# tardis-sn/stardis

Measured on AMD Instinct MI355X. Metric: spectral points/sec (N_nu x N_depth), higher is better.
Workload: dtype f64; 1 GPU; S-c2: solar MARCS structure, 6500-6600 A at R=500000, 2000 lines, fp64; scaling=one GPU, n_nu_global=7634, n_nu_per_gpu=7634, n_depth=56, n_lines=2000, n_theta=20, voigt_evaluations_global=16803184, parallelism=nu-shard x1, hip_graph=False, graph_steps_per_launch=1, syntheses_in_flight_per_gpu=1, line_inputs=dense, outputs=F_nu and total_alphas (N_d, N_nu); the optional alpha_line plane is not written

## Files before the change

stardis_amd/csrc/sdx_kernels.h:

```cpp
#pragma once
#include <type_traits>

#include "sdx_math.h"
#include "sdx_broadening.h"
#include "sdx_cheb.h"

namespace sdx {

constexpr int kBlock = 256;

__device__ __forceinline__ void wave_sync()
{
    __builtin_amdgcn_fence(__ATOMIC_RELEASE, "wavefront");
    __builtin_amdgcn_wave_barrier();
    __builtin_amdgcn_fence(__ATOMIC_ACQUIRE, "wavefront");
}


constexpr int kDnuPartials = 256;
constexpr int kGridSample = 2048;
constexpr int kGridSampleOffset = 512;
__device__ __forceinline__ void grid_sample_block(const int bid, const int n_blocks, int64_t n_nu, const double* __restrict__ nus, double* __restrict__ sample)
{
    const int64_t cstride = (n_nu + kGridSample - 1) / kGridSample;
// ... 159 lines not shown

__device__ __forceinline__ int64_t window_rule(int64_t c, int64_t n_nu, double d_nu, double r_dnu, double gamma, double dw, double alpha,
                                               int& lo, int& hi)
{
    const double pixels = mul_rn(div_by(mul_rn(add_rn(gamma, dw), alpha), d_nu, r_dnu), 20.0);
    const double forced = pixels > 10.0 ? pixels : 10.0;
    const int64_t hw = forced >= (double)n_nu ? n_nu : (int64_t)forced;
    const int64_t l = c - hw, h = c + hw;
    lo = (int)(l < 0 ? 0 : l);
    hi = (int)(h > n_nu ? n_nu : h);
    return hw;
}

constexpr int kPreDepths = 64;
constexpr int kPreBlock = 1024;

constexpr int kNarrowHalfWidth = 64;
constexpr int kNarrowReach = 128;
constexpr int kMediumHalfWidth = 4096;
constexpr int kMaxTile = 512;

#ifdef SDX_WALK_STATS
constexpr int kWalkStatSlots = 1 << 19;
__device__ unsigned long long g_walk_stats[(size_t)kWalkStatSlots * 8];
#endif
#ifdef SDX_PRE_STATS
constexpr int kPreStatSlots = 1 << 14;
__device__ unsigned long long g_pre_stats[(size_t)kPreStatSlots * 8];
#define SDX_PRE_STAMP(n) do { if (tid == 0) pst[n] = wall_clock64(); } while (0)
#else
#define SDX_PRE_STAMP(n) do { } while (0)
#endif
struct alignas(16) WideScan {
    int lo, hi, clo, chi;
};
struct alignas(16) WideRec {
    double lnu, inv, yk, cv, cd, spare;
};
struct alignas(16) WideSlow {
    double y, amp;
};
struct alignas(32) WideRec32 {
    float nuh, yk, inv, ncl, cv, cd, pad0, pad1;
};
struct LineWork {
    WideScan* wscan;
    WideRec* wrec;
    WideSlow* wslow;
    WideRec32* wrec32;
    unsigned char* nhw;
    int skip_unlisted_scan;
    double* n_inv;
    double* n_y;
    double* n_amp;
    int narrow_raw;
    float* n_inv32;
    float* n_y32;
    float* n_amp32;
    float2v* lnu32;
    int* cnt_ge;
    int* centre;
    int* nhw_max;
    int* whw_max;
    int* hlist;
    int* hcount;
    int* xlist;
    int* wlist;
    int* wrank;
    WideScan* hscan;
    const int* sel;
    int n_pix;
    int gather;
    int64_t shard_begin, shard_end;
    unsigned long long* evals;
    int* ticket;
    int front;
    int n_csplit;
    const int* far_range;
};

__device__ __forceinline__ int* wide_list_of(const LineWork& w, int64_t n_lines) { return w.whw_max + n_lines; }
__device__ __forceinline__ int* wide_list_counts(const LineWork& w) { return w.hcount + 16; }

__device__ __forceinline__ unsigned small_div_magic(int d) { return d > 1 ? 0xFFFFFFFFu / (unsigned)d + 1u : 0u; }
__device__ __forceinline__ int small_div(int k, unsigned magic) { return magic ? (int)__umulhi((unsigned)k, magic) : k; }

constexpr int kListMaxChunks = kGridSample - 8;
__device__ __forceinline__ void compact_wide_lines(const LineWork& w, const int64_t n_lines, unsigned long long* __restrict__ s_mask, const int tid)
{
    const int n_split = w.n_csplit;
    const int n_chunks = (int)((n_lines + 63) >> 6);
    const int wave = tid >> 6, lane = tid & 63;
    int* const s_tot = reinterpret_cast<int*>(s_mask + kListMaxChunks);
    int* const clist = wide_list_of(w, n_lines);
    int* const ccount = wide_list_counts(w);
    for (int q = wave; q < n_chunks; q += kPreBlock / 64) {
        const int64_t l = (int64_t)q * 64 + lane;
        const unsigned long long m = __ballot(l < n_lines && w.whw_max[l] > 0);
        if (lane == 0) s_mask[q] = m;
    }
    __syncthreads();
    auto below = [&](int s, int q) {
        int c = 0;
        for (int j = lane; s + j * n_split < q; j += 64) c += __popcll(s_mask[s + j * n_split]);
        for (int off = 32; off > 0; off >>= 1) c += __shfl_xor(c, off);
        return c;
    };
    if (wave < n_split) {
        const int t = below(wave, n_chunks);
        if (lane == 0) s_tot[wave] = t;
    }
    __syncthreads();
    for (int q = wave; q < n_chunks; q += kPreBlock / 64) {
        const int s = q % n_split;
        int base = below(s, q);
        for (int k = 0; k < s; ++k) base += s_tot[k];
        const unsigned long long m = s_mask[q];
        if ((m >> lane) & 1)
            clist[base + (int)__builtin_amdgcn_mbcnt_hi((unsigned)(m >> 32), __builtin_amdgcn_mbcnt_lo((unsigned)m, 0u))] = q * 64 + lane;
    }
    if (tid < n_split) {
        int off = 0;
        for (int k = 0; k < tid; ++k) off += s_tot[k];
        ccount[tid] = s_tot[tid];
        ccount[8 + tid] = off;
    }
}

template <bool GEN, int kPreLines, bool LIST = true>
__device__ __forceinline__ void prepass_block(const int bx, const int by, const int gy, int n_depth, int64_t n_nu, const double* __restrict__ nus,
                                                         const double* __restrict__ dnu_partial, int n_partial,
                                                         int64_t n_lines, const double* __restrict__ line_nus,
                                                         const double* __restrict__ doppler,
                                                         const double* __restrict__ gammas, int gamma_cols,
                                                         const double* __restrict__ alphas, LineWork w,
                                                         int* __restrict__ out_lo_ref, int* __restrict__ out_hi_ref,
                                                         int n_line_blocks, const LineParams& lp, const int tid = threadIdx.x)
{
    int gbx = -1;
    if (bx >= n_line_blocks) {
        if (bx >= n_line_blocks + w.n_pix) {
            if (!w.gather) return;
            gbx = bx - n_line_blocks - w.n_pix;
        } else {
            if (by == 0 && w.cnt_ge) {
                const int64_t pidx = (int64_t)(bx - n_line_blocks) * blockDim.x + tid;
                const bool needed = !w.sel || (pidx >= w.shard_begin - kMediumHalfWidth - 2 * kNarrowReach - kMaxTile &&
                                               pidx <= w.shard_end + kMediumHalfWidth + 2 * kNarrowReach + kMaxTile);
                if (pidx <= n_nu + 1 && needed) {
                    int64_t cnt;
                    if (pidx == 0) cnt = n_lines;
                    else if (pidx == n_nu + 1) cnt = 0;
                    else {
                        const double v = nus[pidx - 1];
                        int64_t lo = 0, hi = n_lines;
                        while (lo < hi) {
                            const int64_t mid = lo + ((hi - lo) >> 1);
                            if (line_nus[mid] <= v) lo = mid + 1; else hi = mid;
                        }
                        cnt = lo;
                    }
                    w.cnt_ge[pidx] = (int)cnt;
                }
            }
            return;
        }
    }
// ... 2900 lines not shown
        const double2* pP = sP + gi + gc - j0;
        const double* pR = sRT + th * rstride + gc - j0;
        const double2 q0 = pP[j0], q1 = pP[j0 + 1];
        double a1 = q1.y, s1 = q1.x;
        double d10 = q0.x - s1;
        double t0 = mul_rn(q0.y * a1, pR[j0]);
#pragma unroll
        for (int j = 0; j < LMAX; ++j) {
            c[j] = 1.0, e[j] = 0.0;
            if (j >= j0) {
                if (j < LMAX - 1 || seg < NS - 1) {
                    const double2 q2 = pP[j + 2];
                    const double s2 = q2.x, a2 = q2.y;
                    const double t1 = mul_rn(a1 * a2, pR[j + 1]);
                    const double d21 = s2 - s1;
                    redo |= rt_coef_fast<false>(t0, t1, d10, d21, s1, c[j], e[j], kc);
                    t0 = t1, d10 = -d21, s1 = s2, a1 = a2;
                } else {
                    redo |= rt_coef_fast<true>(t0, 0.0, d10, 0.0, s1, c[j], e[j], kc);
                }
                A *= c[j];
                B = fma(c[j], B, e[j]);
            }
        }
    }
    if (redo) {
        A = 1.0, B = 0.0;
        for (int j = j0; j < LMAX; ++j) {
            const int gap = gc + j - j0;
            const double s0 = sP[gi + gap].x, s1 = sP[gi + gap + 1].x;
            const double t0 = mul_rn(sP[gi + gap].y * sP[gi + gap + 1].y, sRT[th * rstride + gap]);
            double cj, ej;
            if (gap < n_gap - 1) {
                const double t1 = mul_rn(sP[gi + gap + 1].y * sP[gi + gap + 2].y, sRT[th * rstride + gap + 1]);
                rt_coef_reference<false>(t0, t1, s0 - s1, sP[gi + gap + 2].x - s1, s1, cj, ej);
            } else {
                rt_coef_reference<true>(t0, 0.0, s0 - s1, 0.0, s1, cj, ej);
            }
            A *= cj;
            B = fma(cj, B, ej);
#pragma unroll
            for (int k = 0; k < LMAX; ++k)
                if (k == j) c[k] = cj, e[k] = ej;
        }
    }
    sAB[(seg * 64 + lane) * 2] = A;
    sAB[(seg * 64 + lane) * 2 + 1] = B;
    __syncthreads();
    double inten = 0.0;
    for (int k = 0; k < seg; ++k) inten = fma(sAB[(k * 64 + lane) * 2], inten, sAB[(k * 64 + lane) * 2 + 1]);
    if (seg == 0) {
        if (valid && I_nus) I_nus[(size_t)i * theta_stride + th] = 0.0;
        if (valid && g == 0 && F) F[i] = 0.0;
    }
    double* fx = sFx + (size_t)seg * LMAX * gpw * G + (active ? grp * G + g : 0);
    double* ip = valid && I_nus ? I_nus + ((size_t)(g_lo + 1) * n_nu + i) * theta_stride + th : nullptr;
    const size_t istep = (size_t)n_nu * theta_stride;
#pragma unroll
    for (int j = 0; j < LMAX; ++j) {
        if (j >= j0) {
            inten = fma(c[j], inten, e[j]);
            if (ip) *ip = inten, ip += istep;
            if (active) fx[(j - j0) * gpw * G] = inten * wt;
        }
    }
    fx = sFx + (size_t)seg * LMAX * gpw * G;
    wave_sync();
    if (F) {
        const int half = (n_theta + 1) >> 1;
        for (int p = lane; p < 2 * count * gpw; p += 64) {
            const int h = p & 1, q = p >> 1;
            const int b = (int)(((float)q + 0.5f) * (1.0f / (float)gpw)), gq = q - b * gpw;
            const double* cc = fx + q * G + (h ? half : 0);
            const int cnt = h ? n_theta - half : half;
            double sum = 0.0;
            for (int t = 0; t < cnt; ++t) sum = add_rn(sum, cc[t]);
            const double other = __shfl_xor(sum, 1);
            const int64_t iq = i0 + gq;
            if (h == 0 && iq < n_nu) F[(size_t)(g_lo + b + 1) * fld + iq] = add_rn(sum, other);
        }
    }
}

template <int P>
__global__ __launch_bounds__(kRtBlock) void k_raytrace_cont(int n_depth, int64_t n_nu, int n_theta, int theta_stride, int G,
                                                          const double* __restrict__ nus, const double* __restrict__ temps,
                                                          const double* __restrict__ ray_dist, const double* __restrict__ wts,
                                                          double* __restrict__ F, int64_t fld, double* __restrict__ Fc, int64_t fcld,
                                                          double* __restrict__ I_nus, int inward, int gpw, FusedTotal ft)
{
    constexpr int kBatch = P == 1 ? 4 : 2;
    extern __shared__ double smem[];
    const int lane = threadIdx.x & 63, wave = __builtin_amdgcn_readfirstlane(threadIdx.x >> 6);
    const int grp = lane / G, g = lane - grp * G;
    const int TH = P * G;
    const int64_t i0 = ((int64_t)blockIdx.x * (kRtBlock / 64) + wave) * gpw;
    const int64_t i = i0 + grp;
    const bool active = grp < gpw;
    const bool valid = active && i < n_nu;
    const int64_t ic = i < n_nu ? i : n_nu - 1;
    const int n_gap = n_depth - 1;
    const int col = n_depth;
    double* wbase = smem + (size_t)wave * ((3 * gpw * col + 2 * kBatch * gpw * TH + 1) & ~1);
    double2* sP = (double2*)wbase;
    double* sC = wbase + 2 * gpw * col;
    double* sX = sC + gpw * col;
    double* sXc = sX + kBatch * gpw * TH;
    const double nu = nus[ic];

    if (active) {
        for (int d = g; d < n_depth; d += G) {
            const double ac = ft.cont[(size_t)d * ft.cld + ic];
            double a = ac;
            if (ft.planes) {
                double line = ft.planes[(size_t)d * ft.pld + ic];
                for (int sp = 1; sp < ft.n_planes; ++sp) line = add_rn(line, ft.planes[((size_t)sp * n_depth + d) * ft.pld + ic]);
                a = add_rn(a, line);
                if (valid && ft.line_out) ft.line_out[(size_t)d * ft.out_ld + i] = line;
            }
            for (int x = 0; x < ft.n_extra; ++x) a = add_rn(a, ft.extra[x][(size_t)d * ft.eld + ic]);
            if (valid && ft.total_out) ft.total_out[(size_t)d * ft.out_ld + i] = a;
            sP[grp * col + d] = double2{ft.source ? ft.source[(size_t)d * ft.sld + ic] : planck_staged(nu, temps[d]), sqrt(a)};
            sC[grp * col + d] = sqrt(ac);
        }
    }
    wave_sync();
    const RtConst kc = rt_const_literals();

    const int gi = (active ? grp : 0) * col;
    double inten[P], intc[P], wt[P];
    int th[P];
    bool on[P];
#pragma unroll
    for (int k = 0; k < P; ++k) {
        th[k] = min(g + k * G, n_theta - 1);
        on[k] = g + k * G < n_theta;
        inten[k] = 0.0, intc[k] = 0.0;
        wt[k] = on[k] ? wts[th[k]] : 0.0;
    }
    if (inward) {
        for (int gap = n_gap - 1; gap >= 0; --gap) {
            const int gm = gap > 0 ? gap - 1 : n_gap - 1;
            const int dm = gap > 0 ? gap - 1 : n_depth - 1;
            const double2 q0 = sP[gi + gap + 1], q1 = sP[gi + gap], q2 = sP[gi + dm];
            const double s0 = q0.x, s1 = q1.x, s2 = q2.x;
            const double mg = q1.y * q0.y, mm = sP[gi + gm].y * sP[gi + gm + 1].y;
            const double mgc = sC[gi + gap] * sC[gi + gap + 1], mmc = sC[gi + gm] * sC[gi + gm + 1];
#pragma unroll
            for (int k = 0; k < P; ++k) {
                const double rg = ray_dist[(size_t)gap * theta_stride + th[k]], rm = ray_dist[(size_t)gm * theta_stride + th[k]];
                const double tg = mul_rn(mg, rg), tm = mul_rn(mm, rm);
                const double tgc = mul_rn(mgc, rg), tmc = mul_rn(mmc, rm);
                double c, e, cc, ec;
                rt_coef<false>(tg, tm, s0 - s1, s2 - s1, s1, c, e, kc);
                rt_coef<false>(tgc, tmc, s0 - s1, s2 - s1, s1, cc, ec, kc);
                inten[k] = tm == 0.0 ? inten[k] : fma(c, inten[k], e);
                intc[k] = tmc == 0.0 ? intc[k] : fma(cc, intc[k], ec);
            }
        }
#pragma unroll
        for (int k = 0; k < P; ++k) {
            if (valid && I_nus && on[k]) I_nus[(size_t)i * theta_stride + th[k]] = inten[k];
            if (active) sX[grp * TH + k * G + g] = inten[k] * wt[k], sXc[grp * TH + k * G + g] = intc[k] * wt[k];
        }
        wave_sync();
        if (lane < gpw && i0 + lane < n_nu) {
// ... 235 lines not shown
```

stardis_amd/csrc/stardis_hip.hip:

```cpp
#include <hip/hip_runtime.h>

#include <algorithm>
#include <cmath>
#include <cstdio>
#include <cstdlib>
#include <cstring>
#include <map>
#include <mutex>
#include <string>
#include <unordered_map>
#include <vector>

#include <dlfcn.h>
#include <rccl/rccl.h>

#include <memory>
#include <thread>

#include "../../include/stardis_hip.h"
#include "sdx_kernels.h"

using namespace sdx;

namespace {
// ... 321 lines not shown
        fail(SDX_ERR_HIP, "hipSetDevice failed: no usable HIP device " + std::to_string(device));
        (void)hipGetLastError();
        return nullptr;
    }
    sdx_ctx* ctx = new sdx_ctx();
    ctx->device = device;
    if (hipDeviceGetAttribute(&ctx->n_cu, hipDeviceAttributeMultiprocessorCount, device) != hipSuccess || ctx->n_cu <= 0) ctx->n_cu = 256;
    if (stream) {
        ctx->stream = (hipStream_t)stream;
    } else {
        if (hipStreamCreateWithFlags(&ctx->stream, hipStreamNonBlocking) != hipSuccess) {
            fail(SDX_ERR_HIP, "hipStreamCreate failed");
            delete ctx;
            return nullptr;
        }
        ctx->own_stream = true;
    }
    hipEventCreate(&ctx->t0);
    hipEventCreate(&ctx->t1);
    return ctx;
}

void sdx_destroy(sdx_ctx* ctx)
{
    if (!ctx) return;
    hipSetDevice(ctx->device);
    hipStreamSynchronize(ctx->stream);
    for (auto& r : ctx->records) {
        hipEventDestroy(r.start);
        hipEventDestroy(r.stop);
    }
    for (auto e : ctx->event_pool) hipEventDestroy(e);
    if (ctx->cont_ws) hipFree(ctx->cont_ws);
    if (ctx->t0) hipEventDestroy(ctx->t0);
    if (ctx->t1) hipEventDestroy(ctx->t1);
    if (ctx->line_ws) hipFree(ctx->line_ws);
    if (ctx->small_ws) hipFree(ctx->small_ws);
    if (ctx->part_ws) hipFree(ctx->part_ws);
    if (ctx->far_ws) hipFree(ctx->far_ws);
    if (ctx->cnt_ws) hipFree(ctx->cnt_ws);
    if (ctx->io_dev) hipFree(ctx->io_dev);
    if (ctx->io_pin) hipHostFree(ctx->io_pin);
    if (ctx->xfer_pin) hipHostFree(ctx->xfer_pin);
    for (auto& b : ctx->free_blocks) hipFree(b.second);
    if (ctx->own_stream) hipStreamDestroy(ctx->stream);
    delete ctx;
}

int sdx_set_stream(sdx_ctx* ctx, void* stream)
{
    REQUIRE(ctx, "null context");
    HIP_TRY(hipStreamSynchronize(ctx->stream));
    if (ctx->own_stream) {
        hipStreamDestroy(ctx->stream);
        ctx->own_stream = false;
    }
    if (stream) {
        ctx->stream = (hipStream_t)stream;
    } else {
        HIP_TRY(hipStreamCreateWithFlags(&ctx->stream, hipStreamNonBlocking));
        ctx->own_stream = true;
    }
    return SDX_OK;
}

void* sdx_get_stream(sdx_ctx* ctx) { return ctx ? (void*)ctx->stream : nullptr; }

int sdx_set_int_option(sdx_ctx* ctx, const char* name, int64_t value)
{
    REQUIRE(ctx && name, "sdx_set_int_option: null pointer");
    if (std::strcmp(name, "indexed_min_lines") == 0) {
        ctx->indexed_min_lines = value;
        return SDX_OK;
    }
    if (std::strcmp(name, "prepass_ticket_min_blocks") == 0) {
        ctx->prepass_ticket_min_blocks = value;
        return SDX_OK;
    }
    if (std::strcmp(name, "mixed_precision") == 0) {
        ctx->mixed_precision = value ? 1 : 0;
        return SDX_OK;
    }
    if (std::strcmp(name, "segmented_raytrace") == 0) {
        ctx->segmented_raytrace = value < 0 ? -1 : (value ? 1 : 0);
        return SDX_OK;
    }
    if (std::strcmp(name, "far_field") == 0) {
        ctx->far_field = value < 0 ? -1 : (value ? 1 : 0);
        return SDX_OK;
    }
    if (std::strcmp(name, "wide_list") == 0) {
        ctx->wide_list = value < 0 ? -1 : (value ? 1 : 0);
        return SDX_OK;
    }
    if (std::strcmp(name, "narrow_records") == 0) {
        ctx->narrow_records = value < 0 ? -1 : (value ? 1 : 0);
        return SDX_OK;
    }
    return fail(SDX_ERR_ARG, std::string("unknown option ") + name);
}

static bool far_field_on(const sdx_ctx* ctx, int64_t n_nu_global);
int sdx_far_field_active(const sdx_ctx* ctx, int64_t n_nu_global)
{
    REQUIRE(ctx, "null context");
    return far_field_on(ctx, n_nu_global) ? 1 : 0;
}

int sdx_far_field_rule(int64_t* min_points, int* tile_points, int* near_points)
{
    if (min_points) *min_points = 32768;
    if (tile_points) *tile_points = kFarTile;
    if (near_points) *near_points = (int)(kFarRatio * (kFarTile / 2)) + kFarTile / 2;
    return SDX_OK;
}

int sdx_synchronize(sdx_ctx* ctx)
{
    REQUIRE(ctx, "null context");
    HIP_TRY(hipStreamSynchronize(ctx->stream));
    return SDX_OK;
}

constexpr size_t kBlockPoolLimit = (size_t)4 << 30;
static size_t block_capacity(size_t bytes)
{
    if (bytes <= 256) return 256;
    if (bytes >= ((size_t)1 << 20)) return (bytes + ((size_t)1 << 20) - 1) & ~(((size_t)1 << 20) - 1);
    size_t c = 256;
    while (c < bytes) c <<= 1;
    return c;
}

void* sdx_malloc(sdx_ctx* ctx, size_t bytes)
{
    if (!ctx) return nullptr;
    hipSetDevice(ctx->device);
    const size_t cap = block_capacity(bytes);
    std::lock_guard<std::mutex> lock(ctx->pool_mutex);
    auto it = ctx->free_blocks.lower_bound(cap);
    if (it != ctx->free_blocks.end() && it->first <= 2 * cap) {
        void* p = it->second;
        ctx->free_block_bytes -= it->first;
        ctx->live_blocks[p] = it->first;
        ctx->free_blocks.erase(it);
        return p;
    }
    void* p = nullptr;
    hipError_t e = hipMalloc(&p, cap);
    if (e != hipSuccess && !ctx->free_blocks.empty()) {
        hipStreamSynchronize(ctx->stream);
        for (auto& b : ctx->free_blocks) hipFree(b.second);
        ctx->free_blocks.clear();
        ctx->free_block_bytes = 0;
        e = hipMalloc(&p, cap);
    }
    if (e != hipSuccess) {
        fail(SDX_ERR_OOM, std::string("hipMalloc: ") + hipGetErrorString(e));
        return nullptr;
    }
    ctx->live_blocks[p] = cap;
    return p;
}

int sdx_free(sdx_ctx* ctx, void* ptr)
{
    REQUIRE(ctx, "null context");
// ... 185 lines not shown
    return SDX_OK;
}

int sdx_timer_stop(sdx_ctx* ctx, double* elapsed_ms)
{
    REQUIRE(ctx && elapsed_ms, "sdx_timer_stop: null pointer");
    HIP_TRY(hipEventRecord(ctx->t1, ctx->stream));
    HIP_TRY(hipEventSynchronize(ctx->t1));
    float ms = 0.f;
    HIP_TRY(hipEventElapsedTime(&ms, ctx->t0, ctx->t1));
    *elapsed_ms = ms;
    return SDX_OK;
}

int sdx_profile_enable(sdx_ctx* ctx, int on)
{
    REQUIRE(ctx, "null context");
    ctx->profile = on != 0;
    return SDX_OK;
}

int sdx_profile_reset(sdx_ctx* ctx)
{
    REQUIRE(ctx, "null context");
    HIP_TRY(hipStreamSynchronize(ctx->stream));
    for (auto& r : ctx->records) {
        ctx->event_pool.push_back(r.start);
        ctx->event_pool.push_back(r.stop);
    }
    ctx->records.clear();
    return SDX_OK;
}

int sdx_profile_get(sdx_ctx* ctx, const char* kernel, int64_t* launches, double* total_ms)
{
    REQUIRE(ctx && kernel && launches && total_ms, "sdx_profile_get: null pointer");
    HIP_TRY(hipStreamSynchronize(ctx->stream));
    int64_t n = 0;
    double tot = 0.0;
    for (auto& r : ctx->records) {
        if (std::strcmp(r.name, kernel) != 0) continue;
        float ms = 0.f;
        HIP_TRY(hipEventElapsedTime(&ms, r.start, r.stop));
        tot += ms;
        ++n;
    }
    *launches = n;
    *total_ms = tot;
    return SDX_OK;
}

int sdx_profile_variant(sdx_ctx* ctx, const char* kernel, char* out, int out_len)
{
    REQUIRE(ctx && kernel && out && out_len > 0, "sdx_profile_variant: null pointer");
    out[0] = 0;
    for (auto& r : ctx->records)
        if (std::strcmp(r.name, kernel) == 0 && r.variant) std::snprintf(out, (size_t)out_len, "%s", r.variant);
    return SDX_OK;
}

struct ContinuumJob {
    const sdx_continuum* cont;
    int64_t nu_begin, nu_count;
    double* plane;
};
struct ClassifyPhase {
    int phase;
    int64_t begin, count;
    double* m_max;
};

static const int kSegWaves = knob("SDX_RT_NS") && std::atoi(knob("SDX_RT_NS")) == 4 ? 4 : 8;
static const int kSegMax = kSegWaves == 4 ? 14 : 7;
static int lane_recip(int G)
{
    return 65536 / G + 1;
}
static size_t seg_lds_doubles(int n_depth, int nth)
{
    const int gpw = 64 / nth;
    return (size_t)kSegWaves * 128 + std::max((((size_t)nth * ((n_depth - 1) | 1) + 1) & ~(size_t)1) + (size_t)2 * gpw * n_depth, (size_t)kSegWaves * kSegMax * gpw * nth);
}
constexpr int64_t kSegLegacyWaves = (int64_t)3 * 4 * 256;
static bool use_segmented_raytrace(const sdx_ctx* ctx, int n_depth, int64_t n_nu_global, int n_theta, bool plain)
{
    static const int env_mode = knob("SDX_RT_SEG") ? std::atoi(knob("SDX_RT_SEG")) : -1;
    const int mode = ctx->segmented_raytrace >= 0 ? (int)ctx->segmented_raytrace : env_mode;
    if (mode == 0 || !plain || n_theta > 64) return false;
    if ((n_depth - 1 + kSegWaves - 1) / kSegWaves > kSegMax || seg_lds_doubles(n_depth, n_theta) * sizeof(double) > 64 * 1024) return false;
    if (mode == 1) return true;
    const int64_t legacy_waves = (n_nu_global + 64 / n_theta - 1) / (64 / n_theta);
    return legacy_waves < kSegLegacyWaves;
}

static void launch_line_lists(sdx_ctx* ctx, int64_t n_lines, LineWork& w, int pre_lines, const ClassSource* from_classification = nullptr)
{
    ClassSource cs{};
    if (from_classification) cs = *from_classification;
    else cs.whw_max = w.whw_max;
    w.hlist = w.whw_max + n_lines;
    w.wlist = w.hlist + n_lines;
    w.wrank = w.wlist + n_lines;
    w.xlist = w.sel ? w.wrank + n_lines + 1 : nullptr;
    const unsigned hb = (unsigned)((n_lines + kHlistBlock - 1) / kHlistBlock);
    int* block_cnt = w.hcount + 16;
    hipLaunchKernelGGL(k_hlist_count, dim3(hb), dim3(kHlistBlock), 0, ctx->stream, n_lines, cs, block_cnt, w.sel, pre_lines, w.ticket);
    hipLaunchKernelGGL(k_hlist_scatter, dim3(hb), dim3(kHlistBlock), 0, ctx->stream, n_lines, cs, (const int*)block_cnt, w.hlist,
                       w.wlist, w.wrank, w.hcount, w.xlist, w.sel, pre_lines);
}

static int line_prepass(sdx_ctx* ctx, int n_depth, int64_t n_nu, const double* nus, int64_t n_lines, const double* line_nus,
                        const double* doppler, const double* gammas, int gamma_cols, const double* alphas, bool fill_work,
                        int32_t* lo_ref, int32_t* hi_ref, LineWork* w_out, bool count_evals = true,
                        const ContinuumJob* job = nullptr, const LineParams* gen = nullptr, int64_t nu_begin = 0, int64_t nu_count = -1,
                        const ClassifyPhase* ph = nullptr, int wide_splits = 0)
{
    if (nu_count < 0) nu_count = n_nu;
    const LineParams lp = gen ? *gen : LineParams{};
    int n_partial = 0;
    const bool consumes_classified = ph && ph->phase == 2;
    if (!consumes_classified) ctx->classified.valid = false;
    int rc = ensure_small(ctx, kSmallHeader);
    if (rc) return rc;
    const bool scan_in_block = n_nu <= 16384;
    LineWork w{};
    int pre_lines = ((n_lines + 15) / 16) * ((n_depth + kPreDepths - 1) / kPreDepths) <= 2 * (int64_t)ctx->n_cu ? 16 : 32;
    static const bool no_cull_early = knob("SDX_NO_CULL") != nullptr;
    static const int pre_lines_env = knob("SDX_PRE_LINES") ? std::atoi(knob("SDX_PRE_LINES")) : 0;
    const bool will_cull = fill_work && !no_cull_early && n_lines >= ctx->indexed_min_lines && !count_evals && !gen && n_nu > 16384 && nu_count < n_nu;
    if (will_cull && !lo_ref && (n_lines + 31) / 32 < ctx->prepass_ticket_min_blocks)
        pre_lines = (pre_lines_env == 32 || pre_lines_env == 48) ? pre_lines_env : (n_depth <= 56 ? 54 : 48);
    const int n_line_blocks = (int)((n_lines + pre_lines - 1) / pre_lines);
    int n_pixel_blocks = 0;
    if (fill_work) {
        rc = ensure(ctx, &ctx->line_ws, &ctx->line_ws_bytes, line_ws_need(n_depth, n_lines));
        if (rc) return rc;
        ctx->cnt_ge_len = (size_t)(n_nu + 2 + 63) / 64 * 64;
        rc = ensure(ctx, &ctx->cnt_ws, &ctx->cnt_ws_bytes, (ctx->cnt_ge_len + 10 * (size_t)n_lines + 128 + 3 * ((size_t)n_lines / 1024 + 8) + 8) * sizeof(int));
        if (rc) return rc;
        w = carve(ctx, n_depth, n_lines);
        if (n_depth > kPreDepths) HIP_TRY(hipMemsetAsync(w.nhw_max, 0, (size_t)2 * n_lines * sizeof(int), ctx->stream));
        if (count_evals) HIP_TRY(hipMemsetAsync(w.evals, 0, sizeof(unsigned long long), ctx->stream));
        else w.evals = nullptr;
        n_pixel_blocks = (int)((n_nu + 2 + kPreBlock - 1) / kPreBlock);
    }
    w.sel = nullptr;
    w.gather = 0;
    w.ticket = nullptr;
    w.front = 0;
    const int64_t chunks_per_subset = wide_splits > 0 ? ((n_lines + 63) / 64 + wide_splits - 1) / wide_splits : 0;
    if (fill_work && wide_splits > 0 && (ctx->wide_list == 1 || (ctx->wide_list < 0 && chunks_per_subset >= kListAutoChunks)) &&
        !ctx->mixed_precision && n_lines > 0 && n_lines < ctx->indexed_min_lines && (n_lines + 63) / 64 <= kListMaxChunks) {
        w.n_csplit = wide_splits;
    }
    static const int narrow_records_env = knob("SDX_NARROW_RECORDS") ? std::atoi(knob("SDX_NARROW_RECORDS")) : -1;
    const int narrow_records = ctx->narrow_records >= 0 ? (int)ctx->narrow_records : narrow_records_env;
    const bool very_dense = 2 * n_lines >= 8 * n_nu;
    if (fill_work && !gen && !ctx->mixed_precision && n_lines >= ctx->indexed_min_lines && (narrow_records == 0 || (very_dense && narrow_records != 1))) {
        w.narrow_raw = gamma_cols > 1 ? n_depth : 1;
        w.n_inv = const_cast<double*>(doppler);
        w.n_y = const_cast<double*>(gammas);
        w.n_amp = const_cast<double*>(alphas);
    }
    w.skip_unlisted_scan = (fill_work && n_lines >= ctx->indexed_min_lines && n_depth <= kPreDepths) ? 1 : 0;
    w.n_pix = n_pixel_blocks;
    w.shard_begin = nu_begin;
    w.shard_end = nu_begin + nu_count;
    static const bool no_cull = knob("SDX_NO_CULL") != nullptr;
    const bool cull = fill_work && !no_cull && n_lines >= ctx->indexed_min_lines && !count_evals && !gen && !scan_in_block && nu_count < n_nu;
    REQUIRE(!ph || cull, "two-collective mode is for frequency shards of long dense line lists (>= indexed_min_lines lines, a grid of more than "
                         "16384 points, nu_count < n_nu, no evaluation count)");
    int* const sel = cull ? w.hcount + 4 : nullptr;
    if (cull) n_partial = (int)std::min<int64_t>(kDnuPartials, std::max<int64_t>(1, (n_nu + kBlock * 4 - 1) / (kBlock * 4)));
// ... 912 lines not shown
                         double* Fc = nullptr, int64_t fcld = 0);

int sdx_raytrace_dev(sdx_ctx* ctx, int n_depth, int64_t n_nu, int n_theta, const double* nus, const double* temps,
                     const double* ray_dist, const double* wts, const double* alphas, int64_t ald, double* F, int64_t fld,
                     double* I_nus, int accumulate)
{
    return raytrace_impl(ctx, n_depth, n_nu, n_theta, nus, temps, ray_dist, wts, alphas, ald, F, fld, I_nus, accumulate, 0);
}

int sdx_raytrace_source_dev(sdx_ctx* ctx, int n_depth, int64_t n_nu, int n_theta, const double* nus, const double* temps,
                            const double* ray_dist, const double* wts, const double* alphas, int64_t ald, const double* source,
                            int64_t source_ld, double* F, int64_t fld, double* I_nus, int accumulate, int inward,
                            double photospheric_correction)
{
    REQUIRE(ctx && (n_nu == 0 || !source || source_ld >= n_nu), "raytrace: bad source plane");
    FusedTotal ft{};
    ft.source = source;
    ft.sld = source_ld;
    int rc = raytrace_impl(ctx, n_depth, n_nu, n_theta, nus, temps, ray_dist, wts, alphas, ald, F, fld, I_nus, accumulate, inward ? 1 : 0,
                           source ? &ft : nullptr);
    if (rc || !inward || !F || n_nu == 0) return rc;
    {
        LaunchScope ls(ctx, "k_scale");
        hipLaunchKernelGGL(k_scale, grid2(n_nu, n_depth), dim3(kBlock), 0, ctx->stream, n_depth, n_nu, F, fld, photospheric_correction);
    }
    return check_launch("k_scale");
}

int sdx_raytrace_spherical_dev(sdx_ctx* ctx, int n_depth, int64_t n_nu, int n_theta, const double* nus, const double* temps,
                               const double* ray_dist, const double* wts, const double* alphas, int64_t ald, double* F,
                               int64_t fld, double* I_nus, int accumulate, double photospheric_correction)
{
    int rc = raytrace_impl(ctx, n_depth, n_nu, n_theta, nus, temps, ray_dist, wts, alphas, ald, F, fld, I_nus, accumulate, 1);
    if (rc || !F || n_nu == 0) return rc;
    {
        LaunchScope ls(ctx, "k_scale");
        hipLaunchKernelGGL(k_scale, grid2(n_nu, n_depth), dim3(kBlock), 0, ctx->stream, n_depth, n_nu, F, fld, photospheric_correction);
    }
    return check_launch("k_scale");
}

static int raytrace_impl(sdx_ctx* ctx, int n_depth, int64_t n_nu, int n_theta, const double* nus, const double* temps,
                         const double* ray_dist, const double* wts, const double* alphas, int64_t ald, double* F, int64_t fld,
                         double* I_nus, int accumulate, int inward, const FusedTotal* fused, int64_t nu_global, double* Fc, int64_t fcld)
{
    if (nu_global < n_nu) nu_global = n_nu;
    FusedTotal ft{};
    if (fused) ft = *fused;
    REQUIRE(ctx && n_depth >= 2 && n_nu >= 0 && n_theta > 0, "raytrace: need n_depth >= 2, n_theta > 0");
    if (n_nu == 0) return SDX_OK;
    REQUIRE(nus && temps && ray_dist && wts && ((alphas && ald >= n_nu) || ft.cont), "raytrace: null pointer");
    REQUIRE(!ft.cont || n_theta <= 64, "raytrace: the fused total needs all angles in one launch");
    REQUIRE(!ft.source || n_theta <= 64, "raytrace: a caller-provided source plane needs all angles in one launch");
    REQUIRE((F && fld >= n_nu) || I_nus, "raytrace: no output requested");
    REQUIRE(!Fc || ft.cont, "raytrace: the continuum flux needs a fused total");
    REQUIRE(!Fc || (F && fcld >= n_nu && !accumulate), "raytrace: the continuum flux needs F_nu and continuum_ld >= the columns");
    REQUIRE(!Fc || !ctx->mixed_precision, "raytrace: no continuum flux with mixed_precision = 1 (the fp32 formal solution has no continuum chain)");
    constexpr int kMaxChunk = 64;
    for (int th0 = 0; th0 < n_theta; th0 += kMaxChunk) {
        const int nth = std::min(kMaxChunk, n_theta - th0);
        const double* rd = ray_dist + th0;
        const double* w = wts + th0;
        double* inus = I_nus ? I_nus + th0 : nullptr;
        const int acc = (accumulate || th0 > 0) ? 1 : 0;
        int P = 1;
        if (const char* e = knob("SDX_RT_P")) {
            const int v = std::atoi(e);
            if (v == 1 || v == 2 || v == 4) P = v;
        }
        const int G = (nth + P - 1) / P;
        const int kbatch = P == 1 ? 4 : 2;
        auto lds_bytes = [&](int groups) {
            return ((size_t)(kRtBlock / 64) * (2 * (size_t)groups * n_depth + (size_t)kbatch * groups * P * G)) * sizeof(double);
        };
        int gpw = 64 / G;
        while (gpw > 1 && lds_bytes(gpw) > 64 * 1024) --gpw;
        const size_t shmem = lds_bytes(gpw);
        const unsigned blocks = (unsigned)((n_nu + (int64_t)gpw * (kRtBlock / 64) - 1) / ((int64_t)gpw * (kRtBlock / 64)));
        const unsigned blocks_basic = (unsigned)((n_nu + (int64_t)(64 / G) * (kBlock / 64) - 1) / ((int64_t)(64 / G) * (kBlock / 64)));
        const int seg_gpw = 64 / nth;
        const size_t seg_doubles = seg_lds_doubles(n_depth, nth);
        const unsigned seg_wg = (unsigned)((n_nu + seg_gpw - 1) / seg_gpw), seg_per_xcd = (seg_wg + 7) / 8, seg_blocks = seg_per_xcd * 8;
        if (use_segmented_raytrace(ctx, n_depth, nu_global, n_theta, P == 1 && !inward && !acc)) {
            {
                LaunchScope ls(ctx, "k_raytrace", kSegWaves == 4 ? "k_raytrace_seg<4,14>" : "k_raytrace_seg<8,7>");
#define SDX_SEG_ARGS n_depth, n_nu, nth, n_theta, nus, temps, rd, w, alphas, ald, F, fld, inus, seg_gpw, lane_recip(nth), seg_wg, seg_per_xcd, ft
                if (kSegWaves == 4) hipLaunchKernelGGL((k_raytrace_seg<4, 14>), dim3(seg_blocks), dim3(256), seg_doubles * sizeof(double), ctx->stream, SDX_SEG_ARGS);
                else hipLaunchKernelGGL((k_raytrace_seg<8, 7>), dim3(seg_blocks), dim3(512), seg_doubles * sizeof(double), ctx->stream, SDX_SEG_ARGS);
#undef SDX_SEG_ARGS
            }
            int rc = check_launch("k_raytrace_seg");
            if (rc) return rc;
            if (Fc) {
                FusedTotal fc{};
                fc.cont = ft.cont, fc.cld = ft.cld, fc.source = ft.source, fc.sld = ft.sld;
                {
                    LaunchScope ls(ctx, "k_raytrace", kSegWaves == 4 ? "k_raytrace_seg<4,14> (continuum)" : "k_raytrace_seg<8,7> (continuum)");
#define SDX_SEG_ARGS n_depth, n_nu, nth, n_theta, nus, temps, rd, w, nullptr, 0, Fc, fcld, nullptr, seg_gpw, lane_recip(nth), seg_wg, seg_per_xcd, fc
                    if (kSegWaves == 4) hipLaunchKernelGGL((k_raytrace_seg<4, 14>), dim3(seg_blocks), dim3(256), seg_doubles * sizeof(double), ctx->stream, SDX_SEG_ARGS);
                    else hipLaunchKernelGGL((k_raytrace_seg<8, 7>), dim3(seg_blocks), dim3(512), seg_doubles * sizeof(double), ctx->stream, SDX_SEG_ARGS);
#undef SDX_SEG_ARGS
                }
                if ((rc = check_launch("k_raytrace_seg"))) return rc;
            }
            continue;
        }
        if (ctx->mixed_precision && P == 1 && !inward && !acc && !inus && F && n_theta <= 64) {
            const int g32 = 64 / G;
            const size_t shmem32 = ((((size_t)(n_depth - 1) * nth + 2 * (size_t)n_depth + 3) & ~(size_t)3) +
                                    (size_t)(kRtBlock / 64) * (4 * (size_t)g32 * n_depth + kRt32Batch * (size_t)g32 * G)) * sizeof(float);
            if (shmem32 <= 64 * 1024) {
                {
                    LaunchScope ls(ctx, "k_raytrace", "k_raytrace_f32");
                    const unsigned blocks32 = (unsigned)((n_nu + (int64_t)g32 * (kRtBlock / 64) - 1) / ((int64_t)g32 * (kRtBlock / 64)));
                    hipLaunchKernelGGL(k_raytrace_f32, dim3(blocks32), dim3(kRtBlock), shmem32, ctx->stream, n_depth, n_nu, nth, n_theta, G, nus, temps, rd, w, alphas,
                                       ald, F, fld, g32, ft);
                }
                int rc = check_launch("k_raytrace_f32");
                if (rc) return rc;
                continue;
            }
        }
        if (Fc) {
            REQUIRE(shmem <= 64 * 1024, "raytrace: no continuum flux for models this deep (the columns do not fit LDS)");
            auto lds_cont = [&](int groups) {
                return ((size_t)(kRtBlock / 64) * ((3 * (size_t)groups * n_depth + 2 * (size_t)kbatch * groups * P * G + 1) & ~(size_t)1)) * sizeof(double);
            };
            int gpwc = 64 / G;
            while (gpwc > 1 && lds_cont(gpwc) > 64 * 1024) --gpwc;
            const size_t shmemc = lds_cont(gpwc);
            REQUIRE(shmemc <= 64 * 1024, "raytrace: no continuum flux for models this deep (the columns do not fit LDS)");
            const unsigned blocksc = (unsigned)((n_nu + (int64_t)gpwc * (kRtBlock / 64) - 1) / ((int64_t)gpwc * (kRtBlock / 64)));
            {
                LaunchScope ls(ctx, "k_raytrace", P == 1 ? "k_raytrace_cont<1>" : (P == 2 ? "k_raytrace_cont<2>" : "k_raytrace_cont<4>"));
#define SDX_RTC_ARGS n_depth, n_nu, nth, n_theta, G, nus, temps, rd, w, F, fld, Fc, fcld, inus, inward, gpwc, ft
                if (P == 1) hipLaunchKernelGGL(k_raytrace_cont<1>, dim3(blocksc), dim3(kRtBlock), shmemc, ctx->stream, SDX_RTC_ARGS);
                else if (P == 2) hipLaunchKernelGGL(k_raytrace_cont<2>, dim3(blocksc), dim3(kRtBlock), shmemc, ctx->stream, SDX_RTC_ARGS);
                else hipLaunchKernelGGL(k_raytrace_cont<4>, dim3(blocksc), dim3(kRtBlock), shmemc, ctx->stream, SDX_RTC_ARGS);
#undef SDX_RTC_ARGS
            }
            int rc = check_launch("k_raytrace_cont");
            if (rc) return rc;
            continue;
        }
        {
            LaunchScope ls(ctx, "k_raytrace", shmem <= 64 * 1024 ? (P == 1 ? "k_raytrace<1>" : (P == 2 ? "k_raytrace<2>" : "k_raytrace<4>")) : "k_raytrace_basic");
#define SDX_RT_ARGS n_depth, n_nu, nth, n_theta, G, nus, temps, rd, w, alphas, ald, F, fld, inus, acc
            if (shmem <= 64 * 1024) {
                if (P == 1) hipLaunchKernelGGL(k_raytrace<1>, dim3(blocks), dim3(kRtBlock), shmem, ctx->stream, SDX_RT_ARGS, inward, gpw, ft);
                else if (P == 2) hipLaunchKernelGGL(k_raytrace<2>, dim3(blocks), dim3(kRtBlock), shmem, ctx->stream, SDX_RT_ARGS, inward, gpw, ft);
                else hipLaunchKernelGGL(k_raytrace<4>, dim3(blocks), dim3(kRtBlock), shmem, ctx->stream, SDX_RT_ARGS, inward, gpw, ft);
            } else {
                REQUIRE(!ft.cont && !ft.source, "raytrace: fused total / caller's source plane not available for models this deep");
                REQUIRE(!inward, "raytrace: spherical geometry needs (3*n_depth*64/n_theta + 2*n_depth*n_theta) doubles of LDS per wave; model too deep");
                if (P == 1) hipLaunchKernelGGL(k_raytrace_basic<1>, dim3(blocks_basic), dim3(kBlock), 0, ctx->stream, SDX_RT_ARGS);
                else if (P == 2) hipLaunchKernelGGL(k_raytrace_basic<2>, dim3(blocks_basic), dim3(kBlock), 0, ctx->stream, SDX_RT_ARGS);
                else hipLaunchKernelGGL(k_raytrace_basic<4>, dim3(blocks_basic), dim3(kBlock), 0, ctx->stream, SDX_RT_ARGS);
            }
#undef SDX_RT_ARGS
        }
        int rc = check_launch("k_raytrace");
        if (rc) return rc;
    }
    return SDX_OK;
}

int sdx_raytrace_f64(sdx_ctx* ctx, int n_depth, int64_t n_nu, int n_theta, const double* nus, const double* temps,
                     const double* ray_dist, const double* wts, const double* alphas, double* F, double* I_nus)
{
    REQUIRE(ctx && n_depth >= 2 && n_nu >= 0 && n_theta > 0, "raytrace: need n_depth >= 2, n_theta > 0");
    REQUIRE(n_nu == 0 || (nus && temps && ray_dist && wts && alphas && F), "raytrace: null pointer");
    if (n_nu == 0) return SDX_OK;
    HIP_TRY(hipSetDevice(ctx->device));
    int rc;
    const size_t f8 = sizeof(double), plane = (size_t)n_depth * n_nu * f8;
    const size_t in_bytes[] = {(size_t)n_nu * f8, (size_t)n_depth * f8, (size_t)(n_depth - 1) * n_theta * f8, (size_t)n_theta * f8, plane, plane};
    size_t dev_need = 256, pin_need = HostIo::pad(plane) + 256;
    for (size_t b : in_bytes) dev_need += HostIo::pad(b), pin_need += HostIo::pad(b);
    if (I_nus) dev_need += HostIo::pad(plane * n_theta), pin_need += HostIo::pad(plane * n_theta);
// ... 860 lines not shown
```

Baseline: 5.181 billion spectral points/s.

## Add specialized segmented raytrace step kernel with fused total-opacity staging

Adds a templated k_raytrace_seg_step kernel that stages continuum plus a compile-time number of line planes into LDS, writes total_alphas, and runs the segmented per-depth ray transfer with precomputed geometry (magic division, reciprocals). It replaces the generic segmented kernel when the fused-total shape matches (no source, no extra terms, 0/2/3 planes), including the continuum-flux pass. The aim is to remove runtime branching and generic FusedTotal handling and to cut divisions in the inner loop. The cost is more template instantiations and a new code path whose eligibility conditions must line up with what the old kernel handled.

```diff
diff --git a/stardis_amd/csrc/sdx_kernels.h b/stardis_amd/csrc/sdx_kernels.h
--- a/stardis_amd/csrc/sdx_kernels.h
+++ b/stardis_amd/csrc/sdx_kernels.h
@@ -265,7 +265,7 @@
 __device__ __forceinline__ int* wide_list_of(const LineWork& w, int64_t n_lines) { return w.whw_max + n_lines; }
 __device__ __forceinline__ int* wide_list_counts(const LineWork& w) { return w.hcount + 16; }
 
-__device__ __forceinline__ unsigned small_div_magic(int d) { return d > 1 ? 0xFFFFFFFFu / (unsigned)d + 1u : 0u; }
+__host__ __device__ __forceinline__ unsigned small_div_magic(int d) { return d > 1 ? 0xFFFFFFFFu / (unsigned)d + 1u : 0u; }
 __device__ __forceinline__ int small_div(int k, unsigned magic) { return magic ? (int)__umulhi((unsigned)k, magic) : k; }
 
 constexpr int kListMaxChunks = kGridSample - 8;
@@ -3332,6 +3332,154 @@
     }
 }
 
+struct SegStepGeom {
+    int gpw, g_recip;
+    int per;
+    int L;
+    int rstride;
+    int sp_off;
+    unsigned gpw_magic;
+    unsigned n_wg, per_xcd;
+};
+template <int NS, int LMAX, int N_PLANES, bool KEEP_TOTAL>
+__global__ __launch_bounds__(64 * NS) __attribute__((amdgpu_waves_per_eu(NS >= 8 ? 6 : 4, 8))) void k_raytrace_seg_step(
+    int n_depth, int64_t n_nu, int n_theta, int theta_stride, const double* __restrict__ nus, const double* __restrict__ temps,
+    const double* __restrict__ ray_dist, const double* __restrict__ wts, const double* __restrict__ cont, int64_t cld,
+    const double* __restrict__ planes, int64_t pld, double* __restrict__ total_out, int64_t out_ld, double* __restrict__ F, int64_t fld,
+    SegStepGeom geo)
+{
+    extern __shared__ double smem[];
+    const int lane = threadIdx.x & 63;
+    const int seg = __builtin_amdgcn_readfirstlane(threadIdx.x >> 6);
+    const int G = n_theta, gpw = geo.gpw;
+    const int grp = lane_div(lane, geo.g_recip), g = lane - grp * G;
+    const unsigned wg = (blockIdx.x & 7) * geo.per_xcd + (blockIdx.x >> 3);
+    if ((blockIdx.x >> 3) >= geo.per_xcd || wg >= geo.n_wg) return;
+    const int64_t i0 = (int64_t)wg * gpw;
+    const bool active = grp < gpw;
+    const int n_gap = n_depth - 1, col = n_depth;
+    const int rstride = geo.rstride;
+    double* sAB = smem;
+    double* sRT = sAB + NS * 128;
+    double2* sP = (double2*)(sRT + geo.sp_off);
+    double* sFx = sRT;
+
+    if (grp < geo.per)
+        for (int gp = (NS - 1 - seg) * geo.per + grp; gp < n_gap; gp += NS * geo.per) sRT[g * rstride + gp] = ray_dist[gp * theta_stride + g];
+    const int n_items = n_depth * gpw;
+    if (seg * 64 < n_items) {
+        for (int k = threadIdx.x; k < n_items; k += 64 * NS) {
+            const int d = small_div(k, geo.gpw_magic), gq = k - d * gpw;
+            const int64_t iq = i0 + gq;
+            const bool vq = iq < n_nu;
+            const int64_t ic = vq ? iq : n_nu - 1;
+            const double c0 = cont[(size_t)d * cld + ic];
+            double pl[N_PLANES > 0 ? N_PLANES : 1];
+#pragma unroll
+            for (int sp = 0; sp < N_PLANES; ++sp) pl[sp] = planes[((size_t)sp * n_depth + d) * pld + ic];
+            const double src = planck_staged(nus[ic], temps[d]);
+            double a = c0;
+            if (N_PLANES > 0) {
+                double line = pl[0];
+#pragma unroll
+                for (int sp = 1; sp < N_PLANES; ++sp) line = add_rn(line, pl[sp]);
+                a = add_rn(a, line);
+            }
+            if (KEEP_TOTAL && vq) total_out[(size_t)d * out_ld + iq] = a;
+            sP[gq * col + d] = double2{src, sqrt(a)};
+        }
+    }
+    __syncthreads();
+
+    const int L = geo.L;
+    const int g_end = n_gap - (NS - 1 - seg) * L;
+    const int g_lo = max(0, g_end - L);
+    const int count = max(0, g_end - g_lo);
+    const int j0 = LMAX - count;
+    const int gi = (active ? grp : 0) * col;
+    const int th = min(g, n_theta - 1);
+    const double wt = wts[th];
+    double c[LMAX], e[LMAX];
+    double A = 1.0, B = 0.0;
+    unsigned long long redo = 0;
+    const int gc = count > 0 ? g_lo : 0;
+    const RtConst kc = rt_const_resident();
+    {
+        const double2* pP = sP + gi + gc - j0;
+        const double* pR = sRT + th * rstride + gc - j0;
+        const double2 q0 = pP[j0], q1 = pP[j0 + 1];
+        double a1 = q1.y, s1 = q1.x;
+        double d10 = q0.x - s1;
+        double t0 = mul_rn(q0.y * a1, pR[j0]);
+#pragma unroll
+        for (int j = 0; j < LMAX; ++j) {
+            c[j] = 1.0, e[j] = 0.0;
+            if (j >= j0) {
+                if (j < LMAX - 1 || seg < NS - 1) {
+                    const double2 q2 = pP[j + 2];
+                    const double s2 = q2.x, a2 = q2.y;
+                    const double t1 = mul_rn(a1 * a2, pR[j + 1]);
+                    const double d21 = s2 - s1;
+                    redo |= rt_coef_fast<false>(t0, t1, d10, d21, s1, c[j], e[j], kc);
+                    t0 = t1, d10 = -d21, s1 = s2, a1 = a2;
+                } else {
+                    redo |= rt_coef_fast<true>(t0, 0.0, d10, 0.0, s1, c[j], e[j], kc);
+                }
+                A *= c[j];
+                B = fma(c[j], B, e[j]);
+            }
+        }
+    }
+    if (redo) {
+        A = 1.0, B = 0.0;
+        for (int j = j0; j < LMAX; ++j) {
+            const int gap = gc + j - j0;
+            const double s0 = sP[gi + gap].x, s1 = sP[gi + gap + 1].x;
+            const double t0 = mul_rn(sP[gi + gap].y * sP[gi + gap + 1].y, sRT[th * rstride + gap]);
+            double cj, ej;
+            if (gap < n_gap - 1) {
+                const double t1 = mul_rn(sP[gi + gap + 1].y * sP[gi + gap + 2].y, sRT[th * rstride + gap + 1]);
+                rt_coef_reference<false>(t0, t1, s0 - s1, sP[gi + gap + 2].x - s1, s1, cj, ej);
+            } else {
+                rt_coef_reference<true>(t0, 0.0, s0 - s1, 0.0, s1, cj, ej);
+            }
+            A *= cj;
+            B = fma(cj, B, ej);
+#pragma unroll
+            for (int k = 0; k < LMAX; ++k)
+                if (k == j) c[k] = cj, e[k] = ej;
+        }
+    }
+    sAB[(seg * 64 + lane) * 2] = A;
+    sAB[(seg * 64 + lane) * 2 + 1] = B;
+    __syncthreads();
+    double inten = 0.0;
+    for (int k = 0; k < seg; ++k) inten = fma(sAB[(k * 64 + lane) * 2], inten, sAB[(k * 64 + lane) * 2 + 1]);
+    if (seg == 0 && active && g == 0 && i0 + grp < n_nu) F[i0 + grp] = 0.0;
+    double* fx = sFx + seg * LMAX * gpw * G + (active ? grp * G + g : 0);
+#pragma unroll
+    for (int j = 0; j < LMAX; ++j) {
+        if (j >= j0) {
+            inten = fma(c[j], inten, e[j]);
+            if (active) fx[(j - j0) * gpw * G] = inten * wt;
+        }
+    }
+    fx = sFx + seg * LMAX * gpw * G;
+    wave_sync();
+    const int half = (n_theta + 1) >> 1;
+    for (int p = lane; p < 2 * count * gpw; p += 64) {
+        const int h = p & 1, q = p >> 1;
+        const int b = small_div(q, geo.gpw_magic), gq = q - b * gpw;
+        const double* cc = fx + q * G + (h ? half : 0);
+        const int cnt = h ? n_theta - half : half;
+        double sum = 0.0;
+        for (int t = 0; t < cnt; ++t) sum = add_rn(sum, cc[t]);
+        const double other = __shfl_xor(sum, 1);
+        const int64_t iq = i0 + gq;
+        if (h == 0 && iq < n_nu) F[(size_t)(g_lo + b + 1) * fld + iq] = add_rn(sum, other);
+    }
+}
+
 template <int P>
 __global__ __launch_bounds__(kRtBlock) void k_raytrace_cont(int n_depth, int64_t n_nu, int n_theta, int theta_stride, int G,
                                                           const double* __restrict__ nus, const double* __restrict__ temps,
diff --git a/stardis_amd/csrc/stardis_hip.hip b/stardis_amd/csrc/stardis_hip.hip
--- a/stardis_amd/csrc/stardis_hip.hip
+++ b/stardis_amd/csrc/stardis_hip.hip
@@ -427,7 +427,7 @@
         return SDX_OK;
     }
     if (std::strcmp(name, "segmented_raytrace") == 0) {
-        ctx->segmented_raytrace = value < 0 ? -1 : (value ? 1 : 0);
+        ctx->segmented_raytrace = value < 0 ? -1 : (value >= 2 ? 2 : (value ? 1 : 0));
         return SDX_OK;
     }
     if (std::strcmp(name, "far_field") == 0) {
@@ -779,13 +779,18 @@
     return (size_t)kSegWaves * 128 + std::max((((size_t)nth * ((n_depth - 1) | 1) + 1) & ~(size_t)1) + (size_t)2 * gpw * n_depth, (size_t)kSegWaves * kSegMax * gpw * nth);
 }
 constexpr int64_t kSegLegacyWaves = (int64_t)3 * 4 * 256;
-static bool use_segmented_raytrace(const sdx_ctx* ctx, int n_depth, int64_t n_nu_global, int n_theta, bool plain)
+static int segmented_mode(const sdx_ctx* ctx)
 {
     static const int env_mode = knob("SDX_RT_SEG") ? std::atoi(knob("SDX_RT_SEG")) : -1;
     const int mode = ctx->segmented_raytrace >= 0 ? (int)ctx->segmented_raytrace : env_mode;
+    return mode < 0 ? -1 : std::min(mode, 2);
+}
+static bool use_segmented_raytrace(const sdx_ctx* ctx, int n_depth, int64_t n_nu_global, int n_theta, bool plain)
+{
+    const int mode = segmented_mode(ctx);
     if (mode == 0 || !plain || n_theta > 64) return false;
     if ((n_depth - 1 + kSegWaves - 1) / kSegWaves > kSegMax || seg_lds_doubles(n_depth, n_theta) * sizeof(double) > 64 * 1024) return false;
-    if (mode == 1) return true;
+    if (mode >= 1) return true;
     const int64_t legacy_waves = (n_nu_global + 64 / n_theta - 1) / (64 / n_theta);
     return legacy_waves < kSegLegacyWaves;
 }
@@ -1864,7 +1869,33 @@
         const size_t seg_doubles = seg_lds_doubles(n_depth, nth);
         const unsigned seg_wg = (unsigned)((n_nu + seg_gpw - 1) / seg_gpw), seg_per_xcd = (seg_wg + 7) / 8, seg_blocks = seg_per_xcd * 8;
         if (use_segmented_raytrace(ctx, n_depth, nu_global, n_theta, P == 1 && !inward && !acc)) {
-            {
+            const int step_planes = ft.planes ? ft.n_planes : 0;
+            const bool step_shape = segmented_mode(ctx) != 1 && kSegWaves == 8 && ft.cont && !ft.source && ft.n_extra == 0 && !ft.line_out && !inus && F &&
+                                    (step_planes == 0 || step_planes == 2 || step_planes == 3);
+            SegStepGeom geo{};
+            geo.gpw = seg_gpw, geo.g_recip = lane_recip(nth), geo.per = 64 / nth, geo.L = (n_depth - 1 + kSegWaves - 1) / kSegWaves;
+            geo.rstride = (n_depth - 1) | 1, geo.sp_off = (nth * geo.rstride + 1) & ~1, geo.gpw_magic = small_div_magic(seg_gpw);
+            geo.n_wg = seg_wg, geo.per_xcd = seg_per_xcd;
+            auto launch_step = [&](int planes_n, const double* planes, double* total_out, double* flux, int64_t flux_ld) {
+#define SDX_STEP_LAUNCH(NP, KEEP)                                                                                                              \
+    hipLaunchKernelGGL((k_raytrace_seg_step<8, 7, NP, KEEP>), dim3(seg_blocks), dim3(512), seg_doubles * sizeof(double), ctx->stream, n_depth, n_nu, nth, \
+                       n_theta, nus, temps, rd, w, ft.cont, ft.cld, planes, ft.pld, total_out, ft.out_ld, flux, flux_ld, geo)
+                if (planes_n == 0) {
+                    if (total_out) SDX_STEP_LAUNCH(0, true);
+                    else SDX_STEP_LAUNCH(0, false);
+                } else if (planes_n == 2) {
+                    if (total_out) SDX_STEP_LAUNCH(2, true);
+                    else SDX_STEP_LAUNCH(2, false);
+                } else {
+                    if (total_out) SDX_STEP_LAUNCH(3, true);
+                    else SDX_STEP_LAUNCH(3, false);
+                }
+#undef SDX_STEP_LAUNCH
+            };
+            if (step_shape) {
+                LaunchScope ls(ctx, "k_raytrace", "k_raytrace_seg_step<8,7>");
+                launch_step(step_planes, ft.planes, ft.total_out, F, fld);
+            } else {
                 LaunchScope ls(ctx, "k_raytrace", kSegWaves == 4 ? "k_raytrace_seg<4,14>" : "k_raytrace_seg<8,7>");
 #define SDX_SEG_ARGS n_depth, n_nu, nth, n_theta, nus, temps, rd, w, alphas, ald, F, fld, inus, seg_gpw, lane_recip(nth), seg_wg, seg_per_xcd, ft
                 if (kSegWaves == 4) hipLaunchKernelGGL((k_raytrace_seg<4, 14>), dim3(seg_blocks), dim3(256), seg_doubles * sizeof(double), ctx->stream, SDX_SEG_ARGS);
@@ -1876,7 +1907,10 @@
             if (Fc) {
                 FusedTotal fc{};
                 fc.cont = ft.cont, fc.cld = ft.cld, fc.source = ft.source, fc.sld = ft.sld;
-                {
+                if (segmented_mode(ctx) != 1 && kSegWaves == 8 && !ft.source) {
+                    LaunchScope ls(ctx, "k_raytrace", "k_raytrace_seg_step<8,7> (continuum)");
+                    launch_step(0, nullptr, nullptr, Fc, fcld);
+                } else {
                     LaunchScope ls(ctx, "k_raytrace", kSegWaves == 4 ? "k_raytrace_seg<4,14> (continuum)" : "k_raytrace_seg<8,7> (continuum)");
 #define SDX_SEG_ARGS n_depth, n_nu, nth, n_theta, nus, temps, rd, w, nullptr, 0, Fc, fcld, nullptr, seg_gpw, lane_recip(nth), seg_wg, seg_per_xcd, fc
                     if (kSegWaves == 4) hipLaunchKernelGGL((k_raytrace_seg<4, 14>), dim3(seg_blocks), dim3(256), seg_doubles * sizeof(double), ctx->stream, SDX_SEG_ARGS);
```

Measured after the change: 5.535 billion spectral points/s (median of 6 runs). 1.07x the previous value.
